# google/nerfies

Measured on NVIDIA H100. Metric: ray-samples/sec (coarse+fine, device-timed), higher is better.
Workload: dtype fp16x3 (fp32 emulated on wgmma: 3 fp16 MMA chains, fp32 accumulate)

## Files before the change

nerfies_b200/csrc/field_simt.cuh:

```cuda
#pragma once
#include "common.cuh"

namespace nfb {

constexpr int kTM = 64;
constexpr int kRS = kTM + 4;
constexpr int kKS = 16;
constexpr int kSimtThreads = 256;
constexpr int kSimtSmemFloats =
    2 * kMaxWidth * kRS
    + kMaxIn * kRS
    + 64 * kRS
    + 2 * kKS * kMaxWidth
    + 3 * kTM;
constexpr int kSimtSmemBytes = kSimtSmemFloats * 4;

struct FieldArgs {
  const float* params;
  const float* origins;
  const float* directions;
  const float* z_vals;
  const float* cond;
  const float* window;
  float* samples;
  float* warped;
  long long num_rows;
  int samples_per_ray;
  int use_warp;
  int warp_only;
  int debug;
  float* ray_out;
  float* ray_weights;
  int white_bg, sample_at_infinity;
};

__device__ __forceinline__ void cp_async16(void* smem, const void* gmem) {
  unsigned s = (unsigned)__cvta_generic_to_shared(smem);
  asm volatile("cp.async.cg.shared.global [%0], [%1], 16;\n" ::"r"(s), "l"(gmem));
}
__device__ __forceinline__ void cp_async_commit() {
  asm volatile("cp.async.commit_group;\n" ::);
}
template <int N>
__device__ __forceinline__ void cp_async_wait() {
  asm volatile("cp.async.wait_group %0;\n" ::"n"(N));
}

struct SimtSmem {
  float* buf[2];
  float* in;
  float* out;
  float* slab[2];
  float* wp;
  __device__ float* ptr(int id) const {
    return id == kB0 ? buf[0] : id == kB1 ? buf[1] : id == kOut0 ? out : out + 32 * kRS;
  }
};

template <int NJ>
__device__ __forceinline__ void simt_dense(const Step& st, const float* __restrict__ params,
                                           const SimtSmem& sm) {
  const int tid = threadIdx.x;
  const int lane = tid & 31;
  const int g = tid >> 5;
  const int npad = 32 * NJ;
  const int ktot = st.k_x + st.k_in;
  const float* __restrict__ W = params + st.w_off;
  const float* src = sm.ptr(st.src);
  const float* in = sm.in + st.in_off * kRS;

  float acc[8][NJ];
#pragma unroll
  for (int i = 0; i < 8; ++i)
#pragma unroll
// ... 46 lines not shown
  for (int j = 0; j < NJ; ++j) {
    const int col = lane + 32 * j;
    const float bias = __ldg(params + st.b_off + col);
    float v[8];
#pragma unroll
    for (int i = 0; i < 8; ++i) v[i] = apply_act(acc[i][j] + bias, act);
    float* p = dst + col * kRS + 8 * g;
    *reinterpret_cast<float4*>(p) = make_float4(v[0], v[1], v[2], v[3]);
    *reinterpret_cast<float4*>(p + 4) = make_float4(v[4], v[5], v[6], v[7]);
  }
  __syncthreads();
}

__device__ __forceinline__ void simt_run_net(const Net& net, const float* params,
                                             const SimtSmem& sm) {
  for (int s = 0; s < net.n_steps; ++s) {
    const Step& st = net.steps[s];
    switch (st.npad / 32) {
      case 1: simt_dense<1>(st, params, sm); break;
      case 2: simt_dense<2>(st, params, sm); break;
      case 3: simt_dense<3>(st, params, sm); break;
      case 4: simt_dense<4>(st, params, sm); break;
      case 5: simt_dense<5>(st, params, sm); break;
      case 6: simt_dense<6>(st, params, sm); break;
      case 7: simt_dense<7>(st, params, sm); break;
      default: simt_dense<8>(st, params, sm); break;
    }
  }
}

__global__ void __launch_bounds__(kSimtThreads, 1)
field_simt_kernel(const __grid_constant__ FieldProgram prog, const FieldArgs args) {
  extern __shared__ __align__(16) float smem[];
  SimtSmem sm;
  sm.buf[0] = smem;
  sm.buf[1] = sm.buf[0] + kMaxWidth * kRS;
  sm.in = sm.buf[1] + kMaxWidth * kRS;
  sm.out = sm.in + kMaxIn * kRS;
  sm.slab[0] = sm.out + 64 * kRS;
  sm.slab[1] = sm.slab[0] + kKS * kMaxWidth;
  sm.wp = sm.slab[1] + kKS * kMaxWidth;

  const int tid = threadIdx.x;
  const int r = tid & (kTM - 1);
  const int part = tid >> 6;
  const long long row0 = (long long)blockIdx.x * kTM;
  long long m = row0 + r;
  const bool valid = m < args.num_rows;
  if (!valid) m = args.num_rows - 1;
  const int S = args.samples_per_ray;
  const long long ray = m / S;

  float x[3];
  {
    const float z = args.z_vals ? __ldg(args.z_vals + m) : 0.f;
#pragma unroll
    for (int c = 0; c < 3; ++c)
      x[c] = __ldg(args.origins + ray * 3 + c) + z * __ldg(args.directions + ray * 3 + c);
  }
  const float* cond = args.cond + ray * prog.cond_stride;

  const bool do_warp = args.use_warp && prog.warp_type != 0;
  if (do_warp) {
    const int nf = 6 * prog.Fw;
    if (part == 0) {
#pragma unroll
      for (int c = 0; c < 3; ++c) sm.in[c * kRS + r] = x[c];
    }
    for (int f = part; f < nf; f += 4)
      sm.in[(3 + f) * kRS + r] = __ldg(args.window + f / 6) * posenc_feature(x, f);
    for (int q = part; q < prog.G; q += 4) sm.in[(3 + nf + q) * kRS + r] = __ldg(cond + q);
    __syncthreads();
    simt_run_net(prog.warp, args.params, sm);
    if (part == 0) {
      float h[12], y[3];
#pragma unroll
      for (int q = 0; q < 12; ++q) h[q] = sm.out[q * kRS + r];
      warp_tail(prog.warp_type, h, x, prog.warp_pivot, prog.warp_trans, y);
#pragma unroll
      for (int c = 0; c < 3; ++c) sm.wp[c * kTM + r] = y[c];
      if (args.warped && valid) {
#pragma unroll
        for (int c = 0; c < 3; ++c) args.warped[m * 3 + c] = y[c];
      }
    }
    __syncthreads();
#pragma unroll
    for (int c = 0; c < 3; ++c) x[c] = sm.wp[c * kTM + r];
  } else if (args.warped && valid && part == 0) {
#pragma unroll
    for (int c = 0; c < 3; ++c) args.warped[m * 3 + c] = x[c];
  }
  if (args.warp_only) return;

  {
    const int nf = 6 * prog.Fp;
    if (part == 0) {
#pragma unroll
      for (int c = 0; c < 3; ++c) sm.in[c * kRS + r] = x[c];
    }
    for (int f = part; f < nf; f += 4) sm.in[(3 + f) * kRS + r] = posenc_feature(x, f);
    const int nc = prog.tc + prog.ac + prog.rc;
    for (int q = part; q < nc; q += 4)
      sm.in[(prog.Dp + q) * kRS + r] = __ldg(cond + prog.G + q);
    __syncthreads();
  }
  simt_run_net(prog.nerf, args.params, sm);

  if (part == 0 && valid && args.samples) {
    const float* oa = sm.ptr(prog.alpha_slot);
    const float* orgb = sm.ptr(prog.rgb_slot);
    float4 o;
    o.x = sigmoidf(orgb[0 * kRS + r]);
    o.y = sigmoidf(orgb[1 * kRS + r]);
    o.z = sigmoidf(orgb[2 * kRS + r]);
// ... 7 lines not shown
```

nerfies_b200/csrc/field_tc.cuh:

```cuda
#pragma once
#include "field_simt.cuh"
#include "field_tc3.cuh"
#include "nfb_handle.h"
#include "tc_common.cuh"
#include "tc_program.cuh"

namespace nfb {
namespace tc {

__device__ __forceinline__ void posenc_fast_to_block(uint8_t* block, int r, const float* x, int F,
                                                  const float* __restrict__ window,
                                                  const float* __restrict__ extra, int n_extra,
                                                  int c_begin = 0, int c_end = 8) {
  float feat[64];
#pragma unroll
  for (int k = 0; k < 64; ++k) feat[k] = 0.f;
  float sn[3], cs[3];
#pragma unroll
  for (int c = 0; c < 3; ++c) {
    feat[c] = x[c];
    sincosf(x[c], &sn[c], &cs[c]);
  }
#pragma unroll
  for (int f = 0; f < 10; ++f) {
// ... 117 lines not shown
  static constexpr int kSlotBytes = (kX3 ? 2 : 1) * kABlockBytes;
};
constexpr int kAlphaOff = 14 * kABlockBytes;
constexpr int kScanOff = kAlphaOff + 512;
constexpr int kBarOff = kScanOff + 256;
constexpr int kWgSmemBytes = kBarOff + 256;
static_assert(WgSmem<true>::kRingOff + kWgSlots * WgSmem<true>::kSlotBytes == kAlphaOff &&
              WgSmem<false>::kRingOff + kWgSlots * WgSmem<false>::kSlotBytes == kAlphaOff,
              "each precision's ring ends where the alpha partials begin");
static_assert(kWgSmemBytes <= 232448, "shared memory");

template <bool kX3, int N>
__device__ __forceinline__ void wg_layer_unit(float* d, int src, uint32_t a_hi, uint32_t in_lo, const uint32_t* lo,
                                              uint32_t b_hi, uint32_t b_lo, uint32_t accumulate) {
  if constexpr (kX3) {
    switch (src) {
      case 0: wg_unit<true, N>(d, a_hi, lo + x3_lo_reg(0, 0, 0), b_hi, b_lo, accumulate); break;
      case 1: wg_unit<true, N>(d, a_hi, lo + x3_lo_reg(1, 0, 0), b_hi, b_lo, accumulate); break;
      case 2: wg_unit<true, N>(d, a_hi, lo + x3_lo_reg(2, 0, 0), b_hi, b_lo, accumulate); break;
      case 3: wg_unit<true, N>(d, a_hi, lo + x3_lo_reg(3, 0, 0), b_hi, b_lo, accumulate); break;
      default: wg_unit<true, N>(d, a_hi, in_lo, b_hi, b_lo, accumulate); break;
    }
  } else {
    wg_unit<false, N>(d, a_hi, 0u, b_hi, b_lo, accumulate);
  }
}

struct WgBars {
  uint64_t full[4];
  uint64_t empty[4];
  uint64_t never;
};

template <bool kX3>
__global__ void __launch_bounds__(kWgThreads, 1)
field_wg_kernel(const __grid_constant__ TcProgram prog, const FieldArgs args, const uint8_t* __restrict__ wpack,
                const float* __restrict__ aux, int num_tiles) {
  using Smem = WgSmem<kX3>;
  constexpr int kSlots = kWgSlots, kSlotBytes = Smem::kSlotBytes;
  constexpr int kProducerRegs = kX3 ? 24 : 40, kConsumerRegs = kX3 ? 240 : 232;
  extern __shared__ __align__(1024) uint8_t base[];
  if ((smem_u32(base) & 1023u) != 0) {
    if (threadIdx.x == 0) printf("nfb: dynamic shared memory is not 1024-byte aligned\n");
    __trap();
  }
  WgBars* bars = reinterpret_cast<WgBars*>(base + kBarOff);
  const int tid = threadIdx.x, wg = tid >> 7, warp = tid >> 5, lane = tid & 31;
  if (tid == 0) {
    for (int i = 0; i < kSlots; ++i) { mbar_init(&bars->full[i], 1); mbar_init(&bars->empty[i], 8); }
    mbar_init(&bars->never, 1);
    fence_barrier_init();
  }
  __syncthreads();
  const bool do_warp = args.use_warp && prog.warp_type != 0;
  int first_step = 0;
  if (!do_warp) {
    while (first_step < prog.n_steps && prog.steps[first_step].epi != kEpiWarpHeads) ++first_step;
    first_step = (first_step < prog.n_steps) ? first_step + 1 : 0;
  }
  int last_step = prog.n_steps - 1;
  if (args.warp_only) {
    last_step = 0;
    while (prog.steps[last_step].epi != kEpiWarpHeads) ++last_step;
  }
  const bool fuse = args.ray_out != nullptr && !args.warp_only;
  const int tpr = fuse ? args.samples_per_ray / kTileRows : 1;
  const int groups = num_tiles / tpr;
  const int bid = (int)blockIdx.x;
  const int my_groups = bid < groups ? (groups - bid + (int)gridDim.x - 1) / (int)gridDim.x : 0;
  const int n_my = my_groups * tpr;
  auto tile_of = [&](int i) { return (bid + (i / tpr) * (int)gridDim.x) * tpr + (i % tpr); };

  if (wg == 0) {
    asm volatile("setmaxnreg.dec.sync.aligned.u32 %0;" ::"n"(kProducerRegs));
    if (warp == 0) {
      uint32_t sg = 0, ph = 0, dead = 0;
      if (args.debug & 8) mbar_wait(&bars->never, 0, dead);
      uint8_t* ring = base + Smem::kRingOff;
      for (int ti = 0; ti < n_my; ++ti) {
        for (int si = first_step; si <= last_step; ++si) {
          const TcStep& st = prog.steps[si];
          const uint32_t bytes = (kX3 ? 2u : 1u) * (uint32_t)st.chunk_n * kRowBytes;
          const uint8_t* src = wpack + st.w_off;
          const int n = st.n_chunks * st.nkb;
          for (int u = 0; u < n; ++u) {
            mbar_wait(&bars->empty[sg], ph ^ 1, dead);
            if (!dead && elect_one()) {
              mbar_arrive_expect_tx(&bars->full[sg], bytes);
              bulk_g2s(ring + sg * kSlotBytes, src + (size_t)u * bytes, bytes, &bars->full[sg]);
            }
            __syncwarp();
            if (++sg == kSlots) { sg = 0; ph ^= 1; }
          }
        }
      }
    }
  } else {
    asm volatile("setmaxnreg.inc.sync.aligned.u32 %0;" ::"n"(kConsumerRegs));
    const int cw = wg - 1, t = tid & 127, wq = t >> 5, lq = lane & 3;
    const int arow = 64 * cw + 16 * wq + (lane >> 2);
    const int r = 64 * cw + (t & 63), hs = t >> 6;
    const int cb = hs * 4, ce = cb + 4;
    const int lr = t & 63;
    uint8_t* act_hi = base;
    uint8_t* inh = base + Smem::kInOff;
    uint8_t* inl = inh + kABlockBytes;
    float* alpha_s = reinterpret_cast<float*>(base + kAlphaOff);
    float* scan_s = reinterpret_cast<float*>(base + kScanOff);
    float* scr = reinterpret_cast<float*>(base + cw * 8192);
    const uint32_t rows_off = (uint32_t)cw * 8192u;
    const uint32_t ring_a = smem_u32(base + Smem::kRingOff);
    const uint32_t act_a = smem_u32(act_hi) + rows_off, in_a = smem_u32(inh) + rows_off;
    uint32_t lo[kX3 ? 64 : 1];
    const float alpha_b = __ldg(aux + prog.alpha_b_off);
    const int S = args.samples_per_ray;
    uint32_t sg = 0, ph = 0, dead = 0;
    auto wg_sync = [&]() { asm volatile("bar.sync %0, 128;" ::"r"(1 + cw) : "memory"); };
    RowState row;

    auto begin_tile = [&](int tile) {
      long long m = (long long)tile * kTileRows + r;
      row.valid = m < args.num_rows;
      if (!row.valid) m = args.num_rows - 1;
      row.m = m;
      row.ray = m / S;
      const float z = args.z_vals ? __ldg(args.z_vals + m) : 0.f;
      float org[3], dir[3];
#pragma unroll
      for (int c = 0; c < 3; ++c) {
        dir[c] = __ldg(args.directions + row.ray * 3 + c);
        org[c] = __ldg(args.origins + row.ray * 3 + c);
      }
#pragma unroll
      for (int c = 0; c < 3; ++c) row.x[c] = org[c] + z * dir[c];
      if (fuse) {
        row.z = z;
        row.last = m + 1 == (row.ray + 1) * S;
        const float zn = (!row.last && args.z_vals) ? __ldg(args.z_vals + m + 1) : 0.f;
        const float dnorm = sqrtf(dir[0] * dir[0] + dir[1] * dir[1] + dir[2] * dir[2]);
        const float d = row.last ? (args.sample_at_infinity ? 1e10f : 1e-19f) : (zn - z);
        row.dist = d * dnorm;
      }
      if (!do_warp && args.warped && row.valid && hs == 0) {
#pragma unroll
        for (int c = 0; c < 3; ++c) args.warped[m * 3 + c] = row.x[c];
      }
      const float* cond = args.cond + row.ray * prog.cond_stride;
      encode_input<kX3>(inh, r, hs, row.x, do_warp ? prog.Fw : prog.Fp, do_warp ? args.window : nullptr,
                        do_warp ? cond : cond + prog.G, do_warp ? prog.G : prog.tc);
    };

    float c_T = 1.f, c_cw = 0.f, a_r = 0.f, a_g = 0.f, a_b = 0.f, a_d = 0.f, a_w = 0.f, a_wnl = 0.f, a_med = 0.f;
    if (n_my > 0) begin_tile(tile_of(0));
    fence_proxy_async();
    wg_sync();
    for (int ti = 0; ti < n_my; ++ti) {
      const int tile = tile_of(ti);
      const bool has_next = ti + 1 < n_my;
      for (int si = first_step; si <= last_step; ++si) {
        const TcStep& st = prog.steps[si];
        const float* bias = aux + st.b_off;
        const float inv_s = kX3 ? 1.f / x3_weight_scale(__ldg(aux + prog.scale_off + si)) : 1.f;
        const bool hidden = st.epi == kEpiHidden;
        float acc0[64], acc1[64];
        float* const acc16 = acc0;
        uint32_t prev_sg = 0;
        const int n_units = st.n_chunks * st.nkb;
        for (int u = 0; u < n_units; ++u) {
          const int c = u >= st.nkb ? 1 : 0, kb = u - c * st.nkb;
          const int src = st.src[kb];
          const uint32_t a_hi = src == kSrcIn ? in_a : act_a + (uint32_t)src * kABlockBytes;
          const uint32_t b_hi = ring_a + sg * kSlotBytes, b_lo = b_hi + (uint32_t)st.chunk_n * kRowBytes;
          mbar_wait(&bars->full[sg], ph, dead);
          wg_fence();
          const uint32_t in_lo = in_a + kABlockBytes;
          if (!hidden) wg_layer_unit<kX3, 16>(acc16, src, a_hi, in_lo, lo, b_hi, b_lo, kb);
          else if (c == 0) wg_layer_unit<kX3, 128>(acc0, src, a_hi, in_lo, lo, b_hi, b_lo, kb);
          else wg_layer_unit<kX3, 128>(acc1, src, a_hi, in_lo, lo, b_hi, b_lo, kb);
          wg_commit();
          if (u > 0) {
            wg_wait<1>();
            if (lane == 0) mbar_arrive(&bars->empty[prev_sg]);
          }
          prev_sg = sg;
          if (++sg == kSlots) { sg = 0; ph ^= 1; }
        }
        wg_wait<0>();
// ... 354 lines not shown
```

nerfies_b200/csrc/nfb_api.cu:

```cuda
#include <cuda_runtime.h>

#include <cmath>
#include <cstdarg>
#include <cstdio>
#include <cstring>
#include <cstdlib>
#include <string>
#include <vector>

#include "../../include/nerfies_b200.h"
#include "common.cuh"
#include "nfb_handle.h"
#include "field_simt.cuh"
#include "ray_kernels.cuh"
#include "camera_kernels.cuh"
#include "metrics_kernels.cuh"
#include "tc_common.cuh"
#include "tc_selftest.cuh"
#include "field_tc.cuh"

namespace {

using nfb::FieldProgram;
using nfb::Net;
// ... 243 lines not shown
  easing_window(alpha, F, w);
  NFB_CUDA(cudaMemcpyAsync(h->d_window, w, F * sizeof(float), cudaMemcpyHostToDevice, stream));
  h->h_window_alpha = alpha;
  return 0;
}

int launch_check(nfb_handle* h, const char* what) {
  cudaError_t e = cudaGetLastError();
  if (e != cudaSuccess) return fail("%s launch failed: %s", what, cudaGetErrorString(e));
  h->launches++;
  return 0;
}

int run_cond(nfb_handle* h, int B, const float* viewdirs, const unsigned* warp_id,
             const unsigned* app_id, const unsigned* cam_id, cudaStream_t s, bool encoded = false,
             bool time_encoder = true) {
  const nfb_config& c = h->cfg;
  nfb::CondArgs a{};
  a.viewdirs = viewdirs; a.warp_id = warp_id; a.app_id = app_id; a.cam_id = cam_id;
  a.warp_table = h->d_warp_table; a.app_table = h->d_app_table; a.cam_table = h->d_cam_table;
  a.n_warp = c.num_warp_embeddings; a.n_app = c.num_appearance_embeddings; a.n_cam = c.num_camera_embeddings;
  a.layout = h->cond_layout; a.cond = h->d_cond; a.num_rays = B;
  a.encoded = encoded;
  const nfb::CondLayout& L = h->cond_layout;
  if (L.G + L.tc + L.ac + L.rc() == 0) return 0;
  const long long total = (long long)B * L.stride;
  const int enc = c.warp_field_type != NFB_WARP_NONE ? c.warp_metadata_encoder : NFB_WARP_ENC_GLO;
  if (enc == NFB_WARP_ENC_TIME && !encoded) a.warp_id = nullptr;
  nfb::ray_cond_kernel<<<(unsigned)((total + 255) / 256), 256, 0, s>>>(a);
  if (launch_check(h, "ray_cond_kernel")) return -1;
  if (enc != NFB_WARP_ENC_GLO && !encoded && warp_id && time_encoder) {
    nfb::TimeArgs t{};
    t.params = h->d_packed; t.net = h->time_net;
    t.F = c.time_encoder_num_freqs;
    if (enc == NFB_WARP_ENC_TIME) t.time_f = reinterpret_cast<const float*>(warp_id);
    else t.time_id = warp_id;
    const float alpha = enc == NFB_WARP_ENC_TIME ? h->time_alpha : (float)t.F;
    easing_window(alpha, t.F, t.window);
    t.blend = enc == NFB_WARP_ENC_BLEND; t.time_alpha = h->time_alpha;
    t.cond = h->d_cond; t.stride = L.stride; t.G = L.G; t.num_rays = B;
    nfb::time_embed_kernel<<<(B + nfb::kTimeRays - 1) / nfb::kTimeRays, nfb::kTimeThreads, 0, s>>>(t);
    return launch_check(h, "time_embed_kernel");
  }
  return 0;
}

bool can_fuse_composite(const nfb_handle* h, int S) {
  return h->cfg.precision == NFB_PREC_FP16X3 && S % 128 == 0 && S <= nfb::kMaxSamples;
}

int run_field(nfb_handle* h, int level, long long rows, int S, const float* origins,
              const float* directions, const float* z, float* samples, float* warped,
              bool use_warp, bool warp_only, cudaStream_t s, float* ray_out = nullptr,
              float* ray_weights = nullptr) {
  if (rows == 0) return 0;
  nfb::FieldArgs a{};
  a.ray_out = ray_out; a.ray_weights = ray_weights;
  a.white_bg = h->cfg.use_white_background; a.sample_at_infinity = h->cfg.use_sample_at_infinity;
  a.params = h->d_packed; a.origins = origins; a.directions = directions; a.z_vals = z;
  a.cond = h->d_cond; a.window = h->d_window; a.samples = samples; a.warped = warped;
  a.num_rows = rows; a.samples_per_ray = S; a.use_warp = use_warp; a.warp_only = warp_only;
  a.debug = h->debug_bits;
  const bool prof = h->profiling && !warp_only;
  if (prof) NFB_CUDA(cudaEventRecord(h->ev[level][0], s));
  int rc;
  if (h->cfg.precision == NFB_PREC_FP32) {
    const long long tiles = (rows + nfb::kTM - 1) / nfb::kTM;
    nfb::field_simt_kernel<<<(unsigned)tiles, nfb::kSimtThreads, nfb::kSimtSmemBytes, s>>>(h->prog[level], a);
    rc = launch_check(h, "field_simt_kernel");
  } else {
    rc = nfb::tc::run_field_tc(h, level, a, s);
  }
  if (prof && rc == 0) {
    NFB_CUDA(cudaEventRecord(h->ev[level][1], s));
    h->ev_valid[level] = true;
  }
  return rc;
}

int run_composite(nfb_handle* h, int B, int S, const float* samples, const float* z,
                  const float* directions, float* out, float* weights, cudaStream_t s) {
  if (S > nfb::kMaxSamples) return fail("more than %d samples per ray", nfb::kMaxSamples);
  nfb::CompositeArgs a{};
  a.samples = reinterpret_cast<const float4*>(samples); a.z_vals = z; a.directions = directions;
  a.out = out; a.weights = weights; a.num_rays = B; a.S = S;
  a.white_bg = h->cfg.use_white_background; a.sample_at_infinity = h->cfg.use_sample_at_infinity;
  const int blocks = (B + nfb::kRaysPerBlock - 1) / nfb::kRaysPerBlock;
  const size_t smem = (size_t)nfb::kRaysPerBlock * 3 * S * sizeof(float);
  nfb::composite_kernel<<<blocks, 32 * nfb::kRaysPerBlock, smem, s>>>(a);
  return launch_check(h, "composite_kernel");
}

int run_resample(nfb_handle* h, int B, const float* zc, const float* wc, const float* u_rand,
                 float* zf, cudaStream_t s) {
  const nfb_config& c = h->cfg;
  nfb::ResampleArgs a{};
  a.z_coarse = zc; a.w_coarse = wc; a.u_rand = u_rand; a.u_lin = h->d_ulin; a.z_fine = zf;
  a.num_rays = B; a.nc = c.num_coarse_samples; a.nf = c.num_fine_samples;
  int p = 1;
  while (p < a.nc + a.nf) p <<= 1;
  a.npow2 = p;
  if (a.nc < 3) return fail("hierarchical sampling needs >= 3 coarse samples");
  const int blocks = (B + nfb::kRaysPerBlock - 1) / nfb::kRaysPerBlock;
  const size_t smem = (size_t)nfb::kRaysPerBlock * (2 * a.nc + p) * sizeof(float);
  nfb::resample_kernel<<<blocks, 32 * nfb::kRaysPerBlock, smem, s>>>(a);
  return launch_check(h, "resample_kernel");
}

int render_level(nfb_handle* h, int level, int B, int S, const float* origins, const float* directions,
                 const float* z, bool use_warp, float* out, float* weights, cudaStream_t s) {
  const long long rows = (long long)B * S;
  if (can_fuse_composite(h, S))
    return run_field(h, level, rows, S, origins, directions, z, nullptr, nullptr, use_warp, false, s, out, weights);
  if (run_field(h, level, rows, S, origins, directions, z, h->d_samples, nullptr, use_warp, false, s)) return -1;
  return run_composite(h, B, S, h->d_samples, z, directions, out, weights, s);
}

int* g_abort_host = nullptr;
unsigned long long g_abort_devices = 0;

int ensure_abort_flag() {
  int dev = 0;
  NFB_CUDA(cudaGetDevice(&dev));
  if (!g_abort_host) {
    NFB_CUDA(cudaHostAlloc(&g_abort_host, sizeof(int), cudaHostAllocMapped | cudaHostAllocPortable));
    *g_abort_host = 0;
  }
  if (dev < 64 && !(g_abort_devices >> dev & 1)) {
    int* dptr = nullptr;
    NFB_CUDA(cudaHostGetDevicePointer(&dptr, g_abort_host, 0));
    NFB_CUDA(cudaMemcpyToSymbol(nfb::tc::g_nfb_abort, &dptr, sizeof(dptr)));
    g_abort_devices |= 1ull << dev;
  }
  return 0;
}

int abort_check() {
  if (g_abort_host && *reinterpret_cast<volatile int*>(g_abort_host))
    return fail("a tensor-core kernel aborted: an mbarrier wait timed out (protocol error); its results are invalid "
                "and tensor-core launches are refused until nfb_reset_abort()");
  return 0;
}

int enter_stream(nfb_handle* h, cudaStream_t s) {
  if (h->last_stream_valid && h->last_stream != s) {
    if (!h->ev_order) NFB_CUDA(cudaEventCreateWithFlags(&h->ev_order, cudaEventDisableTiming));
    NFB_CUDA(cudaEventRecord(h->ev_order, h->last_stream));
    NFB_CUDA(cudaStreamWaitEvent(s, h->ev_order, 0));
  }
  h->last_stream = s; h->last_stream_valid = true;
  return 0;
}

int check_call(nfb_handle* h, int B) {
  if (!h) return fail("null handle");
  if (abort_check()) return -1;
  if (!h->params_set) return fail("nfb_set_params has not been called");
  if (B < 0 || B > h->max_rays) return fail("num_rays=%d outside [0, max_rays=%d]", B, h->max_rays);
  return 0;
}

struct MetricsPlan {
  int h[nfb::metrics::kScales], w[nfb::metrics::kScales];
  int tiles_x[nfb::metrics::kScales], tiles_y[nfb::metrics::kScales];
  long long level_off[nfb::metrics::kScales];
  long long part_off[nfb::metrics::kScales];
  int pool_blocks;
  long long err_off, bytes;
// ... 271 lines not shown
  cudaFree(d_map); cudaFree(d_w); cudaFree(d_out); cudaFree(d_max);
  if (e != cudaSuccess) return fail("selftest kernel failed: %s", cudaGetErrorString(e));
  if (out) { out[0] = h_out[0]; out[1] = h_out[1]; }
  return abort_check();
}

int nfb_selftest_gemm(int K, int N, const float* A, const float* W, float* C, void* stream) {
  return selftest_gemm(false, K, N, A, W, C, 1, nullptr, (cudaStream_t)stream);
}

int nfb_selftest_gemm3(int K, int N, const float* A, const float* W, float* C, int reps, long long* out,
                       void* stream) {
  return selftest_gemm(true, K, N, A, W, C, reps, out, (cudaStream_t)stream);
}

int nfb_create(const nfb_config* cfg, int max_rays, nfb_handle** out) {
  if (!cfg || !out) return fail("null argument");
  if (max_rays < 1) return fail("max_rays must be >= 1");
  if (cfg->num_coarse_samples < 2) return fail("num_coarse_samples must be >= 2");
  if (cfg->num_fine_samples < 0) return fail("num_fine_samples must be >= 0");
  if (cfg->precision < NFB_PREC_FP32 || cfg->precision > NFB_PREC_FP16X3) return fail("bad precision");
  int ndev = 0;
  if (cudaGetDeviceCount(&ndev) != cudaSuccess || ndev == 0)
    return fail("no CUDA device: nerfies_b200 has no CPU path");
  nfb_handle* h = new nfb_handle();
  h->cfg = *cfg;
  h->max_rays = max_rays;
  auto bail = [&](int) { nfb_destroy(h); return -1; };
  if (cudaGetDevice(&h->device) != cudaSuccess) return bail(fail("cudaGetDevice failed"));
  cudaDeviceProp prop;
  if (cudaGetDeviceProperties(&prop, h->device) != cudaSuccess) return bail(fail("cudaGetDeviceProperties failed"));
  if (prop.major != 9) return bail(fail("device is sm_%d%d; this library is built for sm_90a only", prop.major, prop.minor));
  h->sm_count = prop.multiProcessorCount;
  if (ensure_abort_flag()) return bail(-1);
  if (build_programs(h)) return bail(-1);
  if (build_tables(h)) return bail(-1);
  const nfb_config& c = h->cfg;
  const int nc = c.num_coarse_samples, nfine = nc + c.num_fine_samples;
  auto dmalloc = [&](float** p, long long n) {
    return cudaMalloc(p, (size_t)std::max<long long>(n, 1) * sizeof(float)) == cudaSuccess ? 0
        : fail("cudaMalloc of %lld floats failed", n);
  };
  const long long B = max_rays;
  if (dmalloc(&h->d_packed, h->packed_floats) ||
      dmalloc(&h->d_warp_table, (long long)c.num_warp_embeddings * c.num_warp_features) ||
      dmalloc(&h->d_app_table, (long long)c.num_appearance_embeddings * c.num_appearance_features) ||
      dmalloc(&h->d_cam_table, (long long)c.num_camera_embeddings * c.num_camera_features) ||
      dmalloc(&h->d_cond, B * h->cond_layout.stride) || dmalloc(&h->d_zc, B * nc) ||
      dmalloc(&h->d_zf, B * nfine) || dmalloc(&h->d_wc, B * nc) ||
      dmalloc(&h->d_samples, B * nfine * 4) || dmalloc(&h->d_out_c, B * 6) ||
      dmalloc(&h->d_out_f, B * 6) || dmalloc(&h->d_in, B * 9))
    return bail(-1);
  if (cudaMalloc(&h->d_ids, (size_t)B * 3 * sizeof(unsigned)) != cudaSuccess) return bail(fail("cudaMalloc ids failed"));
  if (cudaMemset(h->d_packed, 0, (size_t)h->packed_floats * sizeof(float)) != cudaSuccess) return bail(fail("cudaMemset failed"));
  if (cudaFuncSetAttribute(nfb::field_simt_kernel, cudaFuncAttributeMaxDynamicSharedMemorySize,
                           nfb::kSimtSmemBytes) != cudaSuccess)
    return bail(fail("cannot reserve %d bytes of shared memory", nfb::kSimtSmemBytes));
  cudaFuncSetAttribute(nfb::composite_kernel, cudaFuncAttributeMaxDynamicSharedMemorySize, 64 * 1024);
  cudaFuncSetAttribute(nfb::resample_kernel, cudaFuncAttributeMaxDynamicSharedMemorySize, 64 * 1024);
  if (c.precision != NFB_PREC_FP32 && nfb::tc::create_tc(h)) return bail(-1);
  *out = h;
  return 0;
}

void nfb_destroy(nfb_handle* h) {
  if (!h) return;
  nfb::tc::destroy_tc(h);
  float* bufs[] = {h->d_packed, h->d_warp_table, h->d_app_table, h->d_cam_table, h->d_zlin,
                   h->d_lower, h->d_upper, h->d_ulin, h->d_window, h->d_cond, h->d_zc, h->d_zf,
                   h->d_wc, h->d_samples, h->d_out_c, h->d_out_f, h->d_in};
  for (float* p : bufs) if (p) cudaFree(p);
  float* tbufs[] = {h->d_tape, h->d_gpacked, h->d_gwarp, h->d_gapp, h->d_gcam, h->d_dcond, h->d_tr_out, h->d_tr_w, h->d_loss,
                    h->d_ttape, reinterpret_cast<float*>(h->d_sel), h->d_time_tape};
  for (float* p : tbufs) if (p) cudaFree(p);
  if (h->d_ids) cudaFree(h->d_ids);
  for (int l = 0; l < 2; ++l)
    for (int i = 0; i < 2; ++i) if (h->ev[l][i]) cudaEventDestroy(h->ev[l][i]);
  if (h->h_in) cudaFreeHost(h->h_in);
  if (h->h_out) cudaFreeHost(h->h_out);
  if (h->h_ids) cudaFreeHost(h->h_ids);
  if (h->ev_order) cudaEventDestroy(h->ev_order);
  delete h;
}

int nfb_param_count(const nfb_handle* h) { return h ? (int)h->specs.size() : fail("null handle"); }

int nfb_param_info(const nfb_handle* h, int index, char* name, int name_capacity,
                   long long* rows, long long* cols) {
  if (!h) return fail("null handle");
  if (index < 0 || index >= (int)h->specs.size()) return fail("parameter index %d out of range", index);
  const ParamSpec& s = h->specs[index];
  if (name && name_capacity > 0) {
    strncpy(name, s.name.c_str(), name_capacity - 1);
    name[name_capacity - 1] = 0;
  }
  if (rows) *rows = s.rows;
  if (cols) *cols = s.cols;
  return 0;
}

int nfb_set_params(nfb_handle* h, const float* const* tensors, const long long* numels,
                   int count, void* stream) {
  if (!h || !tensors || !numels) return fail("null argument");
  if (count != (int)h->specs.size())
    return fail("expected %d parameter tensors, got %d", (int)h->specs.size(), count);
  cudaStream_t s = (cudaStream_t)stream;
  if (enter_stream(h, s)) return -1;
  for (int i = 0; i < count; ++i) {
    const ParamSpec& p = h->specs[i];
    if (numels[i] != p.rows * p.cols)
      return fail("parameter %d (%s): expected %lld x %lld = %lld elements, got %lld", i,
                  p.name.c_str(), p.rows, p.cols, p.rows * p.cols, numels[i]);
    if (!tensors[i]) return fail("parameter %d (%s) is null", i, p.name.c_str());
    float* base = p.table == 0 ? h->d_packed : p.table == 1 ? h->d_warp_table
                  : p.table == 2 ? h->d_app_table : h->d_cam_table;
    const long long n = p.rows * p.cols;
    if (n == 0) continue;
    pack_kernel<<<(unsigned)((n + 255) / 256), 256, 0, s>>>(tensors[i], base + p.dst_off, p.rows,
                                                            p.cols, p.ld, p.c_off);
    if (launch_check(h, "pack_kernel")) return -1;
  }
  if (h->cfg.precision != NFB_PREC_FP32 && nfb::tc::pack_tc(h, s)) return -1;
  h->params_set = true;
  return 0;
// ... 8 lines not shown
  nfb::coarse_z_kernel<<<(unsigned)((total + 255) / 256), 256, 0, (cudaStream_t)stream>>>(
      h->d_zlin, h->d_lower, h->d_upper, t_rand, z, B, nc);
  return launch_check(h, "coarse_z_kernel");
}

int nfb_sample_pdf(nfb_handle* h, int B, const float* z_coarse, const float* w_coarse,
                   const float* u_rand, float* z_fine, void* stream) {
  if (check_call(h, B)) return -1;
  if (h->cfg.num_fine_samples <= 0) return fail("model has no fine level");
  if (B == 0) return 0;
  if (enter_stream(h, (cudaStream_t)stream)) return -1;
  return run_resample(h, B, z_coarse, w_coarse, u_rand, z_fine, (cudaStream_t)stream);
}

int nfb_render_samples(nfb_handle* h, int level, int B, int S, const float* z_vals,
                       const float* origins, const float* directions, const float* viewdirs,
                       const unsigned* warp_id, const unsigned* app_id, const unsigned* cam_id,
                       float warp_alpha, unsigned flags, float* out, float* weights,
                       float* samples, float* warped_points, void* stream) {
  if (check_call(h, B)) return -1;
  if (level < 0 || level > 1 || (level == 1 && h->cfg.num_fine_samples <= 0)) return fail("bad level %d", level);
  const int smax = h->cfg.num_coarse_samples + h->cfg.num_fine_samples;
  if (S < 1 || (!samples && S > smax)) return fail("num_samples=%d exceeds the workspace (%d)", S, smax);
  if (B == 0) return 0;
  cudaStream_t s = (cudaStream_t)stream;
  if (enter_stream(h, s)) return -1;
  if (set_window(h, warp_alpha, s)) return -1;
  if (run_cond(h, B, viewdirs ? viewdirs : directions, warp_id, app_id, cam_id, s,
               (flags & NFB_FLAG_METADATA_ENCODED) != 0)) return -1;
  float* smp = samples ? samples : h->d_samples;
  const bool use_warp = !(flags & NFB_FLAG_NO_WARP);
  if (run_field(h, level, (long long)B * S, S, origins, directions, z_vals, smp, warped_points,
                use_warp, false, s)) return -1;
  if (out) return run_composite(h, B, S, smp, z_vals, directions, out, weights, s);
  return 0;
}

int nfb_render_forward(nfb_handle* h, int B, const float* origins, const float* directions,
                       const float* viewdirs, const unsigned* warp_id, const unsigned* app_id,
                       const unsigned* cam_id, float warp_alpha, const float* t_rand,
                       const float* u_rand, unsigned flags, float* out_coarse, float* out_fine,
                       float* w_coarse, float* w_fine, float* z_fine, void* stream) {
  if (check_call(h, B)) return -1;
  if (B == 0) return 0;
  const nfb_config& c = h->cfg;
  cudaStream_t s = (cudaStream_t)stream;
  if (enter_stream(h, s)) return -1;
  const int nc = c.num_coarse_samples, nfine = nc + c.num_fine_samples;
  const bool use_warp = !(flags & NFB_FLAG_NO_WARP);
  const bool fine = c.num_fine_samples > 0 && !(flags & NFB_FLAG_COARSE_ONLY);
  if (set_window(h, warp_alpha, s)) return -1;
  if (run_cond(h, B, viewdirs ? viewdirs : directions, warp_id, app_id, cam_id, s,
               (flags & NFB_FLAG_METADATA_ENCODED) != 0)) return -1;
  if (nfb_coarse_z_vals(h, B, t_rand, h->d_zc, stream)) return -1;
  float* wc = w_coarse ? w_coarse : h->d_wc;
  if (render_level(h, 0, B, nc, origins, directions, h->d_zc, use_warp, out_coarse ? out_coarse : h->d_out_c,
                   wc, s)) return -1;
  if (!fine) return 0;
  float* zf = z_fine ? z_fine : h->d_zf;
  if (run_resample(h, B, h->d_zc, wc, u_rand, zf, s)) return -1;
  return render_level(h, 1, B, nfine, origins, directions, zf, use_warp, out_fine ? out_fine : h->d_out_f,
                      w_fine, s);
}

int nfb_render_forward_host(nfb_handle* h, int B, const float* origins, const float* directions,
                            const float* viewdirs, const unsigned* warp_id,
                            const unsigned* app_id, const unsigned* cam_id, float warp_alpha,
                            unsigned flags, float* out_coarse, float* out_fine, void* stream) {
  if (check_call(h, B)) return -1;
  if (flags & NFB_FLAG_METADATA_ENCODED)
    return fail("NFB_FLAG_METADATA_ENCODED is only supported by the device entry points");
  if (B == 0) return 0;
  cudaStream_t s = (cudaStream_t)stream;
  if (enter_stream(h, s)) return -1;
  const size_t mr = h->max_rays;
  if (!h->h_in) NFB_CUDA(cudaMallocHost(&h->h_in, mr * 9 * sizeof(float)));
  if (!h->h_out) NFB_CUDA(cudaMallocHost(&h->h_out, mr * 12 * sizeof(float)));
  if (!h->h_ids) NFB_CUDA(cudaMallocHost(&h->h_ids, mr * 3 * sizeof(unsigned)));
  const size_t n3 = (size_t)B * 3;
  memcpy(h->h_in, origins, n3 * sizeof(float));
  memcpy(h->h_in + mr * 3, directions, n3 * sizeof(float));
  if (viewdirs) memcpy(h->h_in + mr * 6, viewdirs, n3 * sizeof(float));
  const unsigned* ids[3] = {warp_id, app_id, cam_id};
  for (int i = 0; i < 3; ++i)
    if (ids[i]) memcpy(h->h_ids + mr * i, ids[i], (size_t)B * sizeof(unsigned));
  NFB_CUDA(cudaMemcpyAsync(h->d_in, h->h_in, n3 * sizeof(float), cudaMemcpyHostToDevice, s));
  NFB_CUDA(cudaMemcpyAsync(h->d_in + mr * 3, h->h_in + mr * 3, n3 * sizeof(float), cudaMemcpyHostToDevice, s));
  if (viewdirs)
    NFB_CUDA(cudaMemcpyAsync(h->d_in + mr * 6, h->h_in + mr * 6, n3 * sizeof(float), cudaMemcpyHostToDevice, s));
  for (int i = 0; i < 3; ++i)
    if (ids[i])
      NFB_CUDA(cudaMemcpyAsync(h->d_ids + mr * i, h->h_ids + mr * i, (size_t)B * sizeof(unsigned),
                               cudaMemcpyHostToDevice, s));
  if (nfb_render_forward(h, B, h->d_in, h->d_in + mr * 3, viewdirs ? h->d_in + mr * 6 : nullptr,
                         warp_id ? h->d_ids : nullptr, app_id ? h->d_ids + mr : nullptr,
                         cam_id ? h->d_ids + 2 * mr : nullptr, warp_alpha, nullptr, nullptr, flags,
                         h->d_out_c, h->d_out_f, nullptr, nullptr, nullptr, stream))
    return -1;
  const bool fine = h->cfg.num_fine_samples > 0 && !(flags & NFB_FLAG_COARSE_ONLY);
  if (out_coarse)
    NFB_CUDA(cudaMemcpyAsync(h->h_out, h->d_out_c, (size_t)B * 6 * sizeof(float), cudaMemcpyDeviceToHost, s));
  if (out_fine && fine)
    NFB_CUDA(cudaMemcpyAsync(h->h_out + mr * 6, h->d_out_f, (size_t)B * 6 * sizeof(float), cudaMemcpyDeviceToHost, s));
  NFB_CUDA(cudaStreamSynchronize(s));
  if (abort_check()) return -1;
  if (out_coarse) memcpy(out_coarse, h->h_out, (size_t)B * 6 * sizeof(float));
  if (out_fine && fine) memcpy(out_fine, h->h_out + mr * 6, (size_t)B * 6 * sizeof(float));
  return 0;
}

int nfb_warp_forward(nfb_handle* h, int P, const float* points, const unsigned* warp_id,
                     float warp_alpha, unsigned flags, float* warped, void* stream) {
  if (check_call(h, P)) return -1;
  if (h->cfg.warp_field_type == NFB_WARP_NONE) return fail("model has no warp field");
  if (P == 0) return 0;
// ... 11 lines not shown
```

nerfies_b200/csrc/nfb_handle.h:

```cpp
#pragma once
#include <cuda_runtime.h>

#include <cmath>
#include <cstdarg>
#include <cstdio>
#include <cstring>
#include <string>
#include <vector>

#include "../../include/nerfies_b200.h"
#include "common.cuh"
#include "ray_kernels.cuh"
#include "tc_program.cuh"

namespace {

thread_local std::string g_error;

int fail(const char* fmt, ...) {
  char buf[1024];
  va_list ap;
  va_start(ap, fmt);
  vsnprintf(buf, sizeof(buf), fmt, ap);
  va_end(ap);
  g_error = buf;
  return -1;
}

#define NFB_CUDA(expr)                                                        \
  do {                                                                        \
    cudaError_t e_ = (expr);                                                  \
    if (e_ != cudaSuccess)                                                    \
      return fail("%s failed: %s (%s:%d)", #expr, cudaGetErrorString(e_),     \
                  __FILE__, __LINE__);                                        \
  } while (0)

struct ParamSpec {
  std::string name;
  long long rows, cols;
  long long dst_off;
  int ld, c_off;
  int table;
};

__global__ void pack_kernel(const float* __restrict__ src, float* __restrict__ dst,
                            long long rows, long long cols, int ld, int c_off) {
  const long long idx = (long long)blockIdx.x * blockDim.x + threadIdx.x;
  if (idx >= rows * cols) return;
  const long long r = idx / cols, c = idx - r * cols;
  dst[r * ld + c_off + c] = src[idx];
}

int pad32(int n) { return (n + 31) / 32 * 32; }

}

struct nfb_handle {
  nfb_config cfg;
  int max_rays = 0;
  int device = 0;
  nfb::FieldProgram prog[2];
  std::vector<ParamSpec> specs;
  long long packed_floats = 0;
  float* d_packed = nullptr;
  float* d_warp_table = nullptr;
  float* d_app_table = nullptr;
  float* d_cam_table = nullptr;
  bool params_set = false;
  float *d_zlin = nullptr, *d_lower = nullptr, *d_upper = nullptr, *d_ulin = nullptr;
  float* d_window = nullptr;
  float h_window_alpha = NAN;
  float *d_cond = nullptr, *d_zc = nullptr, *d_zf = nullptr, *d_wc = nullptr;
  float* d_samples = nullptr;
  float *d_out_c = nullptr, *d_out_f = nullptr;
  float *d_in = nullptr, *h_in = nullptr, *h_out = nullptr;
  unsigned *d_ids = nullptr, *h_ids = nullptr;
  long long launches = 0;
  bool profiling = false;
  cudaEvent_t ev[2][2] = {{nullptr, nullptr}, {nullptr, nullptr}};
  bool ev_valid[2] = {false, false};
  nfb::CondLayout cond_layout{};
  int sm_count = 132;
  nfb::Net time_net{};
  float time_alpha = 0.f;
  cudaStream_t last_stream = nullptr;
  bool last_stream_valid = false;
  cudaEvent_t ev_order = nullptr;
  float* d_tape = nullptr; long long tape_floats = 0;
  float *d_gpacked = nullptr, *d_gwarp = nullptr, *d_gapp = nullptr, *d_gcam = nullptr;
  float *d_dcond = nullptr, *d_tr_out = nullptr, *d_tr_w = nullptr, *d_loss = nullptr;
  float* d_ttape = nullptr; long long ttape_floats = 0;
  float* d_time_tape = nullptr; long long time_tape_floats = 0;
  int* d_sel = nullptr; long long sel_cap = 0;
  int train_precision = NFB_TRAIN_FP32;
  int debug_bits = 0;
  nfb::tc::TcProgram tcprog[2];
  unsigned char* d_wpack = nullptr;
  float* d_aux = nullptr;
  long long wpack_bytes = 0, aux_floats = 0;
  struct TcPackJob { int level, step, chunk; int simt_w_off, ld, n, n0, k_total; std::vector<int> k_map; };
  std::vector<TcPackJob> tc_jobs;
  struct TcAuxJob { int src_off, count, stride, dst_off; };
  std::vector<TcAuxJob> tc_aux_jobs;
};
```

nerfies_b200/csrc/ray_kernels.cuh:

```cuda
#pragma once
#include <math_constants.h>

#include "../../include/nerfies_b200.h"
#include "common.cuh"

namespace nfb {

struct CondLayout {
  int G, tc, ac, dv, cc;
  int A, C;
  int stride;
  __host__ __device__ int rc() const { return dv + ac + cc; }
};

inline CondLayout cond_layout(const nfb_config& c) {
  CondLayout L{};
  L.G = c.warp_field_type != NFB_WARP_NONE ? c.num_warp_features : 0;
  L.A = c.num_appearance_features;
  L.C = c.num_camera_features;
  L.tc = (c.use_appearance_metadata && c.use_trunk_condition) ? L.A : 0;
  L.ac = (c.use_appearance_metadata && c.use_alpha_condition) ? L.A : 0;
  L.dv = c.use_viewdirs ? 3 + 6 * c.num_nerf_viewdir_freqs : 0;
  L.cc = c.use_camera_metadata ? L.C : 0;
  L.stride = L.G + L.tc + L.ac + L.rc();
// ... 191 lines not shown
  __syncwarp();
  if (lane == 0) {
    float t = 1.0f;
    for (int i = 0; i < S; ++i) {
      cum[i] = t;
      t = t * (1.0f - alpha[i] + 1e-10f);
    }
  }
  __syncwarp();
  float sr = 0.f, sg_ = 0.f, sb = 0.f, sd = 0.f, sa = 0.f, sa_nolast = 0.f;
  for (int i = lane; i < S; i += 32) {
    const float w = alpha[i] * cum[i];
    const float4 c = sg[i];
    sr += w * c.x; sg_ += w * c.y; sb += w * c.z;
    sd += w * zs[i];
    sa += w;
    if (i + 1 < S) sa_nolast += w;
    alpha[i] = w;
    if (a.weights) a.weights[(size_t)ray * S + i] = w;
  }
#pragma unroll
  for (int o = 16; o > 0; o >>= 1) {
    sr += __shfl_xor_sync(0xffffffffu, sr, o);
    sg_ += __shfl_xor_sync(0xffffffffu, sg_, o);
    sb += __shfl_xor_sync(0xffffffffu, sb, o);
    sd += __shfl_xor_sync(0xffffffffu, sd, o);
    sa += __shfl_xor_sync(0xffffffffu, sa, o);
    sa_nolast += __shfl_xor_sync(0xffffffffu, sa_nolast, o);
  }
  __syncwarp();
  if (lane == 0) {
    float c = 0.f, med = 0.f;
    for (int i = 0; i < S; ++i) {
      c += alpha[i];
      if (c >= 0.5f) { med = zs[i]; break; }
    }
    float r = sr, g = sg_, b = sb;
    if (a.white_bg) {
      const float bg = 1.f - sa;
      r = r + bg; g = g + bg; b = b + bg;
    }
    float* o = a.out + (size_t)ray * 6;
    o[0] = r; o[1] = g; o[2] = b; o[3] = sd; o[4] = med;
    o[5] = a.sample_at_infinity ? sa_nolast : sa;
  }
}

struct ResampleArgs {
  const float* z_coarse;
  const float* w_coarse;
  const float* u_rand;
  const float* u_lin;
  float* z_fine;
  int num_rays, nc, nf, npow2;
};

__global__ void __launch_bounds__(32 * kRaysPerBlock)
resample_kernel(const ResampleArgs a) {
  extern __shared__ float sh[];
  const int warp = threadIdx.x >> 5, lane = threadIdx.x & 31;
  const int ray = blockIdx.x * kRaysPerBlock + warp;
  if (ray >= a.num_rays) return;
  const int nc = a.nc, nf = a.nf;
  const int nb = nc - 1;
  float* bins = sh + warp * (2 * nc + a.npow2);
  float* cdf = bins + nc;
  float* zs = cdf + nc;
  const float* zc = a.z_coarse + (size_t)ray * nc;
  const float* wc = a.w_coarse + (size_t)ray * nc;
  for (int i = lane; i < nc; i += 32) zs[i] = zc[i];
  __syncwarp();
  for (int i = lane; i < nb; i += 32) bins[i] = .5f * (zs[i + 1] + zs[i]);
  for (int i = lane; i < nb - 1; i += 32) cdf[i + 1] = wc[i + 1] + 1e-5f;
  __syncwarp();
  if (lane == 0) {
    float total = 0.f;
    for (int i = 1; i < nb; ++i) total += cdf[i];
    float c = 0.f;
    cdf[0] = 0.f;
    for (int i = 1; i < nb; ++i) {
      c += cdf[i] / total;
      cdf[i] = c;
    }
  }
  __syncwarp();
  for (int j = lane; j < nf; j += 32) {
    const float u = a.u_rand ? a.u_rand[(size_t)ray * nf + j] : a.u_lin[j];
    int lo = 0, hi = nb;
    while (lo < hi) {
      const int mid = (lo + hi) >> 1;
      if (cdf[mid] <= u) lo = mid + 1; else hi = mid;
    }
    const int idx = lo - 1;
    const int i0 = min(max(idx, 0), nb - 2);
    const int i1 = min(max(idx + 1, 1), nb - 1);
    const float c0 = cdf[i0], c1 = cdf[i1], b0 = bins[i0], b1 = bins[i1];
    float denom = c1 - c0;
    if (denom < 1e-5f) denom = 1.f;
    const float t = (u - c0) / denom;
    zs[nc + j] = b0 + t * (b1 - b0);
  }
  const int n = nc + nf;
  for (int i = n + lane; i < a.npow2; i += 32) zs[i] = CUDART_INF_F;
  __syncwarp();
  for (int k = 2; k <= a.npow2; k <<= 1) {
    for (int j = k >> 1; j > 0; j >>= 1) {
      for (int i = lane; i < a.npow2; i += 32) {
        const int p = i ^ j;
        if (p > i) {
          const float x = zs[i], y = zs[p];
          const bool up = (i & k) == 0;
          if ((x > y) == up) { zs[i] = y; zs[p] = x; }
        }
      }
      __syncwarp();
    }
  }
  float* out = a.z_fine + (size_t)ray * n;
  for (int i = lane; i < n; i += 32) out[i] = zs[i];
}

}
```

Measured before the change: 119.1 million.

## Reuse coarse warped points in fine pass instead of re-running warp field

The coarse pass now stores its warped sample positions. The resampler emits the new fine z values plus a sort permutation. The fine pass then runs the warp MLP only on the new fine samples, gathers warped points for the merged sorted set, and feeds them to the NeRF field directly, skipping warp recomputation for the coarse samples. This adds extra buffers, a gather kernel and a warp-only launch, and the resampler has to carry indices through its bitonic sort.

```diff
diff --git a/nerfies_b200/csrc/field_simt.cuh b/nerfies_b200/csrc/field_simt.cuh
--- a/nerfies_b200/csrc/field_simt.cuh
+++ b/nerfies_b200/csrc/field_simt.cuh
@@ -20,6 +20,7 @@
   const float* origins;
   const float* directions;
   const float* z_vals;
+  const float* points;
   const float* cond;
   const float* window;
   float* samples;
@@ -172,7 +173,10 @@
   const long long ray = m / S;
 
   float x[3];
-  {
+  if (args.points) {
+#pragma unroll
+    for (int c = 0; c < 3; ++c) x[c] = __ldg(args.points + m * 3 + c);
+  } else {
     const float z = args.z_vals ? __ldg(args.z_vals + m) : 0.f;
 #pragma unroll
     for (int c = 0; c < 3; ++c)
@@ -180,7 +184,7 @@
   }
   const float* cond = args.cond + ray * prog.cond_stride;
 
-  const bool do_warp = args.use_warp && prog.warp_type != 0;
+  const bool do_warp = args.use_warp && prog.warp_type != 0 && !args.points;
   if (do_warp) {
     const int nf = 6 * prog.Fw;
     if (part == 0) {
diff --git a/nerfies_b200/csrc/field_tc.cuh b/nerfies_b200/csrc/field_tc.cuh
--- a/nerfies_b200/csrc/field_tc.cuh
+++ b/nerfies_b200/csrc/field_tc.cuh
@@ -193,7 +193,7 @@
     fence_barrier_init();
   }
   __syncthreads();
-  const bool do_warp = args.use_warp && prog.warp_type != 0;
+  const bool do_warp = args.use_warp && prog.warp_type != 0 && !args.points;
   int first_step = 0;
   if (!do_warp) {
     while (first_step < prog.n_steps && prog.steps[first_step].epi != kEpiWarpHeads) ++first_step;
@@ -272,8 +272,13 @@
         dir[c] = __ldg(args.directions + row.ray * 3 + c);
         org[c] = __ldg(args.origins + row.ray * 3 + c);
       }
-#pragma unroll
-      for (int c = 0; c < 3; ++c) row.x[c] = org[c] + z * dir[c];
+      if (args.points) {
+#pragma unroll
+        for (int c = 0; c < 3; ++c) row.x[c] = __ldg(args.points + m * 3 + c);
+      } else {
+#pragma unroll
+        for (int c = 0; c < 3; ++c) row.x[c] = org[c] + z * dir[c];
+      }
       if (fuse) {
         row.z = z;
         row.last = m + 1 == (row.ray + 1) * S;
diff --git a/nerfies_b200/csrc/nfb_api.cu b/nerfies_b200/csrc/nfb_api.cu
--- a/nerfies_b200/csrc/nfb_api.cu
+++ b/nerfies_b200/csrc/nfb_api.cu
@@ -319,16 +319,17 @@
 int run_field(nfb_handle* h, int level, long long rows, int S, const float* origins,
               const float* directions, const float* z, float* samples, float* warped,
               bool use_warp, bool warp_only, cudaStream_t s, float* ray_out = nullptr,
-              float* ray_weights = nullptr) {
+              float* ray_weights = nullptr, const float* points = nullptr) {
   if (rows == 0) return 0;
   nfb::FieldArgs a{};
   a.ray_out = ray_out; a.ray_weights = ray_weights;
   a.white_bg = h->cfg.use_white_background; a.sample_at_infinity = h->cfg.use_sample_at_infinity;
   a.params = h->d_packed; a.origins = origins; a.directions = directions; a.z_vals = z;
+  a.points = points;
   a.cond = h->d_cond; a.window = h->d_window; a.samples = samples; a.warped = warped;
   a.num_rows = rows; a.samples_per_ray = S; a.use_warp = use_warp; a.warp_only = warp_only;
   a.debug = h->debug_bits;
-  const bool prof = h->profiling && !warp_only;
+  const bool prof = h->profiling && !warp_only && !points;
   if (prof) NFB_CUDA(cudaEventRecord(h->ev[level][0], s));
   int rc;
   if (h->cfg.precision == NFB_PREC_FP32) {
@@ -359,28 +360,60 @@
 }
 
 int run_resample(nfb_handle* h, int B, const float* zc, const float* wc, const float* u_rand,
-                 float* zf, cudaStream_t s) {
+                 float* zf, cudaStream_t s, float* z_new = nullptr, uint16_t* src = nullptr) {
   const nfb_config& c = h->cfg;
   nfb::ResampleArgs a{};
   a.z_coarse = zc; a.w_coarse = wc; a.u_rand = u_rand; a.u_lin = h->d_ulin; a.z_fine = zf;
+  a.z_new = z_new; a.src = src;
   a.num_rays = B; a.nc = c.num_coarse_samples; a.nf = c.num_fine_samples;
   int p = 1;
   while (p < a.nc + a.nf) p <<= 1;
   a.npow2 = p;
   if (a.nc < 3) return fail("hierarchical sampling needs >= 3 coarse samples");
   const int blocks = (B + nfb::kRaysPerBlock - 1) / nfb::kRaysPerBlock;
-  const size_t smem = (size_t)nfb::kRaysPerBlock * (2 * a.nc + p) * sizeof(float);
+  size_t smem = (size_t)nfb::kRaysPerBlock * (2 * a.nc + p) * sizeof(float);
+  if (src) smem += (size_t)nfb::kRaysPerBlock * p * sizeof(uint16_t);
   nfb::resample_kernel<<<blocks, 32 * nfb::kRaysPerBlock, smem, s>>>(a);
   return launch_check(h, "resample_kernel");
 }
 
 int render_level(nfb_handle* h, int level, int B, int S, const float* origins, const float* directions,
-                 const float* z, bool use_warp, float* out, float* weights, cudaStream_t s) {
+                 const float* z, bool use_warp, float* out, float* weights, cudaStream_t s,
+                 float* warped = nullptr, const float* points = nullptr) {
   const long long rows = (long long)B * S;
   if (can_fuse_composite(h, S))
-    return run_field(h, level, rows, S, origins, directions, z, nullptr, nullptr, use_warp, false, s, out, weights);
-  if (run_field(h, level, rows, S, origins, directions, z, h->d_samples, nullptr, use_warp, false, s)) return -1;
+    return run_field(h, level, rows, S, origins, directions, z, nullptr, warped, use_warp, false, s, out, weights,
+                     points);
+  if (run_field(h, level, rows, S, origins, directions, z, h->d_samples, warped, use_warp, false, s, nullptr, nullptr,
+                points))
+    return -1;
   return run_composite(h, B, S, h->d_samples, z, directions, out, weights, s);
+}
+
+bool reuses_warp(const nfb_handle* h, bool use_warp) {
+  return use_warp && h->d_warped_c != nullptr;
+}
+
+int render_fine_reusing_warp(nfb_handle* h, int B, const float* origins, const float* directions,
+                             const float* zf, float* out, float* weights, cudaStream_t s) {
+  const nfb_config& c = h->cfg;
+  const int nc = c.num_coarse_samples, nf = c.num_fine_samples, n = nc + nf;
+  const bool prof = h->profiling;
+  if (prof) NFB_CUDA(cudaEventRecord(h->ev[1][0], s));
+  if (run_field(h, 1, (long long)B * nf, nf, origins, directions, h->d_znew, nullptr, h->d_warped_new, true, true, s))
+    return -1;
+  nfb::GatherWarpedArgs g{};
+  g.warped_c = h->d_warped_c; g.warped_new = h->d_warped_new; g.src = h->d_src; g.warped_fine = h->d_warped_fine;
+  g.num_rays = B; g.nc = nc; g.nf = nf;
+  const long long total = (long long)B * n;
+  nfb::gather_warped_kernel<<<(unsigned)((total + 255) / 256), 256, 0, s>>>(g);
+  if (launch_check(h, "gather_warped_kernel")) return -1;
+  if (render_level(h, 1, B, n, origins, directions, zf, true, out, weights, s, nullptr, h->d_warped_fine)) return -1;
+  if (prof) {
+    NFB_CUDA(cudaEventRecord(h->ev[1][1], s));
+    h->ev_valid[1] = true;
+  }
+  return 0;
 }
 
 int* g_abort_host = nullptr;
@@ -758,6 +791,14 @@
       dmalloc(&h->d_out_f, B * 6) || dmalloc(&h->d_in, B * 9))
     return bail(-1);
   if (cudaMalloc(&h->d_ids, (size_t)B * 3 * sizeof(unsigned)) != cudaSuccess) return bail(fail("cudaMalloc ids failed"));
+  if (c.warp_field_type != NFB_WARP_NONE && c.num_fine_samples > 0) {
+    const int nf = c.num_fine_samples;
+    if (dmalloc(&h->d_warped_c, B * nc * 3) || dmalloc(&h->d_warped_new, B * nf * 3) ||
+        dmalloc(&h->d_warped_fine, B * nfine * 3) || dmalloc(&h->d_znew, B * nf))
+      return bail(-1);
+    if (cudaMalloc(&h->d_src, (size_t)B * nfine * sizeof(uint16_t)) != cudaSuccess)
+      return bail(fail("cudaMalloc of %lld sample indices failed", B * nfine));
+  }
   if (cudaMemset(h->d_packed, 0, (size_t)h->packed_floats * sizeof(float)) != cudaSuccess) return bail(fail("cudaMemset failed"));
   if (cudaFuncSetAttribute(nfb::field_simt_kernel, cudaFuncAttributeMaxDynamicSharedMemorySize,
                            nfb::kSimtSmemBytes) != cudaSuccess)
@@ -774,8 +815,10 @@
   nfb::tc::destroy_tc(h);
   float* bufs[] = {h->d_packed, h->d_warp_table, h->d_app_table, h->d_cam_table, h->d_zlin,
                    h->d_lower, h->d_upper, h->d_ulin, h->d_window, h->d_cond, h->d_zc, h->d_zf,
-                   h->d_wc, h->d_samples, h->d_out_c, h->d_out_f, h->d_in};
+                   h->d_wc, h->d_samples, h->d_out_c, h->d_out_f, h->d_in, h->d_warped_c,
+                   h->d_warped_new, h->d_warped_fine, h->d_znew};
   for (float* p : bufs) if (p) cudaFree(p);
+  if (h->d_src) cudaFree(h->d_src);
   float* tbufs[] = {h->d_tape, h->d_gpacked, h->d_gwarp, h->d_gapp, h->d_gcam, h->d_dcond, h->d_tr_out, h->d_tr_w, h->d_loss,
                     h->d_ttape, reinterpret_cast<float*>(h->d_sel), h->d_time_tape};
   for (float* p : tbufs) if (p) cudaFree(p);
@@ -890,15 +933,20 @@
   if (set_window(h, warp_alpha, s)) return -1;
   if (run_cond(h, B, viewdirs ? viewdirs : directions, warp_id, app_id, cam_id, s,
                (flags & NFB_FLAG_METADATA_ENCODED) != 0)) return -1;
+  const bool reuse = fine && reuses_warp(h, use_warp);
   if (nfb_coarse_z_vals(h, B, t_rand, h->d_zc, stream)) return -1;
   float* wc = w_coarse ? w_coarse : h->d_wc;
   if (render_level(h, 0, B, nc, origins, directions, h->d_zc, use_warp, out_coarse ? out_coarse : h->d_out_c,
-                   wc, s)) return -1;
+                   wc, s, reuse ? h->d_warped_c : nullptr)) return -1;
   if (!fine) return 0;
   float* zf = z_fine ? z_fine : h->d_zf;
+  float* of = out_fine ? out_fine : h->d_out_f;
+  if (reuse) {
+    if (run_resample(h, B, h->d_zc, wc, u_rand, zf, s, h->d_znew, h->d_src)) return -1;
+    return render_fine_reusing_warp(h, B, origins, directions, zf, of, w_fine, s);
+  }
   if (run_resample(h, B, h->d_zc, wc, u_rand, zf, s)) return -1;
-  return render_level(h, 1, B, nfine, origins, directions, zf, use_warp, out_fine ? out_fine : h->d_out_f,
-                      w_fine, s);
+  return render_level(h, 1, B, nfine, origins, directions, zf, use_warp, of, w_fine, s);
 }
 
 int nfb_render_forward_host(nfb_handle* h, int B, const float* origins, const float* directions,
diff --git a/nerfies_b200/csrc/nfb_handle.h b/nerfies_b200/csrc/nfb_handle.h
--- a/nerfies_b200/csrc/nfb_handle.h
+++ b/nerfies_b200/csrc/nfb_handle.h
@@ -73,6 +73,8 @@
   float *d_cond = nullptr, *d_zc = nullptr, *d_zf = nullptr, *d_wc = nullptr;
   float* d_samples = nullptr;
   float *d_out_c = nullptr, *d_out_f = nullptr;
+  float *d_warped_c = nullptr, *d_warped_new = nullptr, *d_warped_fine = nullptr, *d_znew = nullptr;
+  uint16_t* d_src = nullptr;
   float *d_in = nullptr, *h_in = nullptr, *h_out = nullptr;
   unsigned *d_ids = nullptr, *h_ids = nullptr;
   long long launches = 0;
diff --git a/nerfies_b200/csrc/ray_kernels.cuh b/nerfies_b200/csrc/ray_kernels.cuh
--- a/nerfies_b200/csrc/ray_kernels.cuh
+++ b/nerfies_b200/csrc/ray_kernels.cuh
@@ -267,8 +267,30 @@
   const float* u_rand;
   const float* u_lin;
   float* z_fine;
+  float* z_new;
+  uint16_t* src;
   int num_rays, nc, nf, npow2;
 };
+
+template <bool kIdx>
+__device__ __forceinline__ void bitonic_sort(float* keys, uint16_t* idx, int npow2, int lane) {
+  for (int k = 2; k <= npow2; k <<= 1) {
+    for (int j = k >> 1; j > 0; j >>= 1) {
+      for (int i = lane; i < npow2; i += 32) {
+        const int p = i ^ j;
+        if (p > i) {
+          const float x = keys[i], y = keys[p];
+          const bool up = (i & k) == 0;
+          if ((x > y) == up) {
+            keys[i] = y; keys[p] = x;
+            if constexpr (kIdx) { const uint16_t q = idx[i]; idx[i] = idx[p]; idx[p] = q; }
+          }
+        }
+      }
+      __syncwarp();
+    }
+  }
+}
 
 __global__ void __launch_bounds__(32 * kRaysPerBlock)
 resample_kernel(const ResampleArgs a) {
@@ -313,26 +335,42 @@
     float denom = c1 - c0;
     if (denom < 1e-5f) denom = 1.f;
     const float t = (u - c0) / denom;
-    zs[nc + j] = b0 + t * (b1 - b0);
+    const float z = b0 + t * (b1 - b0);
+    zs[nc + j] = z;
+    if (a.z_new) a.z_new[(size_t)ray * nf + j] = z;
   }
   const int n = nc + nf;
   for (int i = n + lane; i < a.npow2; i += 32) zs[i] = CUDART_INF_F;
-  __syncwarp();
-  for (int k = 2; k <= a.npow2; k <<= 1) {
-    for (int j = k >> 1; j > 0; j >>= 1) {
-      for (int i = lane; i < a.npow2; i += 32) {
-        const int p = i ^ j;
-        if (p > i) {
-          const float x = zs[i], y = zs[p];
-          const bool up = (i & k) == 0;
-          if ((x > y) == up) { zs[i] = y; zs[p] = x; }
-        }
-      }
-      __syncwarp();
-    }
-  }
+  uint16_t* si = a.src ? reinterpret_cast<uint16_t*>(sh + kRaysPerBlock * (2 * nc + a.npow2)) + warp * a.npow2
+                       : nullptr;
+  if (si)
+    for (int i = lane; i < a.npow2; i += 32) si[i] = (uint16_t)(i < n ? i : 0);
+  __syncwarp();
+  if (si) bitonic_sort<true>(zs, si, a.npow2, lane);
+  else bitonic_sort<false>(zs, nullptr, a.npow2, lane);
   float* out = a.z_fine + (size_t)ray * n;
   for (int i = lane; i < n; i += 32) out[i] = zs[i];
-}
-
-}
+  if (si)
+    for (int i = lane; i < n; i += 32) a.src[(size_t)ray * n + i] = si[i];
+}
+
+struct GatherWarpedArgs {
+  const float* warped_c;
+  const float* warped_new;
+  const uint16_t* src;
+  float* warped_fine;
+  int num_rays, nc, nf;
+};
+
+__global__ void gather_warped_kernel(const GatherWarpedArgs a) {
+  const int n = a.nc + a.nf;
+  const long long idx = (long long)blockIdx.x * blockDim.x + threadIdx.x;
+  if (idx >= (long long)a.num_rays * n) return;
+  const long long ray = idx / n;
+  const int s = a.src[idx];
+  const float* p = s < a.nc ? a.warped_c + (ray * a.nc + s) * 3 : a.warped_new + (ray * a.nf + (s - a.nc)) * 3;
+  float* o = a.warped_fine + idx * 3;
+  o[0] = p[0]; o[1] = p[1]; o[2] = p[2];
+}
+
+}
```

Result: faster. 125.9 million (median of 6 runs) (+5.7%).
